# valeoai/PAFUSE

Measured on AMD Instinct MI355X. Metric: hypotheses/sec through DDIM loop (H3WB 133-kp, P=20, T=10), higher is better.
Workload: dtype bf16x3 (every fp32 GEMM operand as the exact sum of three bf16 slices, six bf16 MFMA products per fp32-equivalent product, fp32 accumulate; activations, LayerNorm, softmax, attention and everything in memory fp32; the residual stream stored centred on its row means)

## Files before the change

### pafuse_amd/csrc/kernels.hpp

```cpp
#pragma once
#include <hip/hip_runtime.h>
#include <stdint.h>

#include <utility>

namespace pafuse {

typedef float f32x16 __attribute__((ext_vector_type(16)));
typedef float f32x4 __attribute__((ext_vector_type(4)));

constexpr int BK = 32;
constexpr int LDK = 36;

typedef __bf16 bf16x8 __attribute__((ext_vector_type(8)));
__device__ __forceinline__ bf16x8 to_bf16x8(const f32x4 lo, const f32x4 hi) {
    bf16x8 v;
#pragma unroll
    for (int i = 0; i < 4; ++i) v[i] = (__bf16)lo[i], v[4 + i] = (__bf16)hi[i];
    return v;
}

#ifdef PAFUSE_MFMA_K8
typedef __bf16 bf16x4_t __attribute__((ext_vector_type(4)));
typedef short s16x4_t __attribute__((ext_vector_type(4)));
// ... 273 lines not shown
    float* out_head;
    float* ln_stats;
    const float* ln_in;
    const float* ln_s;
    const uint8_t* Ah;
    const uint8_t* Wh;
    uint8_t* out_h;
    uint8_t* out_xh;
    uint8_t* out_nh;
    const uint8_t* resid_h;
    const float* rowscale;
    int rs_temporal, rs_J, rs_FJ;
    float* out_pre;
    unsigned long long* stamps;
};

#ifdef PAFUSE_XQ_FENCE
struct XqFence {
    __device__ __forceinline__ XqFence() {
        if (PAFUSE_XQ_FENCE & 1) __builtin_amdgcn_fence(__ATOMIC_ACQUIRE, "agent");
        if (PAFUSE_XQ_FENCE & 4) {
            __builtin_amdgcn_fence(__ATOMIC_ACQUIRE, "agent");
            asm volatile("s_waitcnt vmcnt(0)" ::: "memory");
            __syncthreads();
        }
    }
    __device__ __forceinline__ ~XqFence() {
        if (PAFUSE_XQ_FENCE & 2) {
            asm volatile("s_waitcnt vmcnt(0)" ::: "memory");
            __builtin_amdgcn_fence(__ATOMIC_RELEASE, "agent");
            asm volatile("s_waitcnt vmcnt(0)" ::: "memory");
        }
    }
};
#define PAFUSE_XQ_GUARD() XqFence xq_fence_guard
#else
#define PAFUSE_XQ_GUARD()
#endif

#ifdef PAFUSE_STAMPS
__device__ __forceinline__ unsigned long long pafuse_stamp() {
    unsigned long long t;
    __builtin_amdgcn_sched_barrier(0);
    asm volatile("s_memtime %0\n\ts_waitcnt lgkmcnt(0)" : "=s"(t)::"memory");
    __builtin_amdgcn_sched_barrier(0);
    return t;
}
#ifndef PAFUSE_STAMP_SLOTS
#define PAFUSE_STAMP_SLOTS 4
#endif
#define PAFUSE_STAMP(i)                                                                         \
    if (p.stamps && (threadIdx.x & 63) == 0)                                                    \
    p.stamps[((size_t)blockIdx.x * (blockDim.x >> 6) + (threadIdx.x >> 6)) * PAFUSE_STAMP_SLOTS + (i)] = pafuse_stamp()
#else
#define PAFUSE_STAMP(i)
#endif

template <int WM, int WN, int NT>
struct GemmTile {
    static constexpr int NTHR = WM * WN * 64;
    static constexpr int BM = WM * 32;
    static constexpr int BN = WN * NT * 32;
    static constexpr int STAGE_FLOATS = (BM + BN) * LDK;
    static constexpr int W_ROW_SPLIT = WSPLIT_ROW_BYTES / 4;
    static constexpr int STAGE_FLOATS_SPLIT = BM * LDK + BN * W_ROW_SPLIT;
};

template <int WN, int NT, int BM, int EPI, int VEC = 0>
__device__ __forceinline__ void epilogue_row_per_lane(f32x16 (&acc)[NT], const GemmParams& p, const int64_t m0, const int n0,
                                                      const int wm, const int wn, const int r, const int h, float* smem,
                                                      const float ws = 1.0f) {
    constexpr int BNV = WN * NT * 32;
    auto vec4 = [&](const float* gptr, int slot, int n) -> f32x4 {
        if constexpr (VEC > 0) return *reinterpret_cast<const f32x4*>(smem + VEC + slot * BNV + (n - n0));
        else return *reinterpret_cast<const f32x4*>(gptr + n);
    };
    const int64_t m = m0 + wm * 32 + r;
    const bool live = m < p.M;
    const int64_t mo = (live ? m : p.M - 1) * p.N;
    const int nb = n0 + wn * NT * 32 + 4 * h;
    if constexpr (EPI == EPI_BIAS) {
        float rstd = 1.0f;
        if (p.ln_in) rstd = p.ln_in[2 * (live ? m : p.M - 1) + 1];
        rstd *= ws;
#pragma unroll
        for (int nt = 0; nt < NT; ++nt)
#pragma unroll
            for (int q = 0; q < 4; ++q) {
                const int n = nb + 32 * nt + 8 * q;
                const f32x4 b4 = *reinterpret_cast<const f32x4*>(p.bias + n);
                f32x4 v;
                if (p.ln_in) {
#pragma unroll
                    for (int e = 0; e < 4; ++e) v[e] = fmaf(rstd, acc[nt][4 * q + e], b4[e]);
                } else {
#pragma unroll
                    for (int e = 0; e < 4; ++e) v[e] = fmaf(acc[nt][4 * q + e], ws, b4[e]);
                }
#pragma unroll
                for (int e = 0; e < 4; ++e)
                    if (p.act) v[e] = gelu_erf(v[e]);
                if (live) *reinterpret_cast<f32x4*>(p.out + mo + n) = v;
            }
        PAFUSE_STAMP(2);
        return;
    } else {
        float* red = smem;
        const float invC = 1.0f / (float)p.N;
// ... 528 lines not shown
        if (m >= p.M) continue;
        float rstd = 1.0f;
        if (p.ln_in) rstd = p.ln_in[2 * m + 1];
        float* const orow = p.out + m * p.N + n0 + 4 * qd;
#pragma unroll
        for (int n = 0; n < NB; ++n) {
            const f32x4 b4 = *reinterpret_cast<const f32x4*>(p.bias + n0 + 16 * n + 4 * qd);
            f32x4 v;
            if (p.ln_in) {
#pragma unroll
                for (int e = 0; e < 4; ++e) v[e] = fmaf(rstd, acc[g][n][e], b4[e]);
            } else {
#pragma unroll
                for (int e = 0; e < 4; ++e) v[e] = acc[g][n][e] + b4[e];
            }
#pragma unroll
            for (int e = 0; e < 4; ++e)
                if (p.act) v[e] = gelu_erf(v[e]);
            if (p.dact_u) {
                const f32x4 u = *reinterpret_cast<const f32x4*>(p.dact_u + m * p.N + n0 + 4 * qd + 16 * n);
#pragma unroll
                for (int e = 0; e < 4; ++e) v[e] *= gelu_erf_grad(u[e]);
            }
            *reinterpret_cast<f32x4*>(orow + 16 * n) = v;
            if (p.out_act) {
#pragma unroll
                for (int e = 0; e < 4; ++e) v[e] = gelu_erf(v[e]);
                *reinterpret_cast<f32x4*>(p.out_act + m * p.N + n0 + 4 * qd + 16 * n) = v;
            }
        }
    }
}

template <int NB, int MINW>
__global__ void __launch_bounds__(256, MINW) gemm16_kernel(const GemmParams p) {
    PAFUSE_XQ_GUARD();
    extern __shared__ __attribute__((aligned(16))) float smem[];
    gemm16_tile<NB>(p, blockIdx.x, gridDim.x, smem);
}

template <int WM, int WN, int NT, int BKC = 32>
struct DmaTile {
    static_assert(BKC == 32 || BKC == 16, "chunk depth");
    static constexpr int NW = WM * WN, NTHR = NW * 64;
    static constexpr int BM = WM * 32, BN = WN * NT * 32;
    static constexpr int A_ROW = BKC * 4, W_ROW = BKC * 6;
    static constexpr int A_BYTES = BM * A_ROW, W_BYTES = BN * W_ROW, STAGE_BYTES = A_BYTES + W_BYTES;
    static constexpr int IA = A_BYTES / 1024, IW = W_BYTES / 1024;
    static constexpr int CNT = (IA + IW + NW - 1) / NW;
    static_assert(W_BYTES % 1024 == 0 && A_BYTES % 1024 == 0, "whole DMA pieces");
    static_assert(BKC == 16 || NW % 2 == 0, "the A swizzle of a wave's DMA lanes must not depend on the instruction index");
};

template <int... Is, class F>
__device__ __forceinline__ void static_for_impl(std::integer_sequence<int, Is...>, F&& f) {
    (f(std::integral_constant<int, Is>{}), ...);
}
template <int N, class F>
__device__ __forceinline__ void static_for(F&& f) {
    static_for_impl(std::make_integer_sequence<int, N>{}, f);
}

template <int OFF>
__device__ __forceinline__ u32x4 lds_read128(uint32_t addr) {
    u32x4 v;
    asm volatile("ds_read_b128 %0, %1 offset:%2" : "=v"(v) : "v"(addr), "i"(OFF));
    return v;
}

template <int N>
__device__ __forceinline__ void wait_vmcnt() {
    static_assert(N >= 0 && N < 64, "vmcnt immediate");
    asm volatile("s_waitcnt vmcnt(%0)" ::"n"(N) : "memory");
}

template <int WN, int NT, int BM, int NW, int NTH, bool HRES, int NSLICE = 2>
__device__ __forceinline__ void epilogue_rows_h(f32x16 (&acc)[NT], const GemmParams& p, const int64_t m0, const int n0, const int wm,
                                                const int wn, const int r, const int h, const int wave, const int lane, float* smem,
                                                const float ws);

template <int WM, int WN, int NT, int EPI, int NSTAGE, int ABL = 0, int BKC = 32, bool SLAB = true>
__device__ __forceinline__ void gemm_dma_tile(const GemmParams& p, const int b, const int nb, float* smem) {
    using T = DmaTile<WM, WN, NT, BKC>;
    constexpr int NW = T::NW, BM = T::BM, BN = T::BN, CNT = T::CNT, IA = T::IA, IW = T::IW;
    constexpr int NS2 = BKC / 16;
    constexpr int RPI = 1024 / T::A_ROW;
    constexpr int CPR = T::A_ROW / 16;
    static_assert(NSTAGE >= 2 && NSTAGE <= 4, "ring depth");
    static_assert(CNT * (NSTAGE - 1) < 64, "vmcnt range");
    uint8_t* const lds = reinterpret_cast<uint8_t*>(smem);
    const uint32_t lds0 = (uint32_t)(size_t)(__attribute__((address_space(3))) void*)smem;

    const int tid = threadIdx.x, lane = tid & 63;
    const int wave = __builtin_amdgcn_readfirstlane(tid >> 6);
    const int wm = wave / WN, wn = wave % WN;
    const int r = lane & 31, h = lane >> 5;
    const int tiles_n = p.N / BN;
    int tile;
    {
        const int xcd = b & 7, q = nb >> 3, rem = nb & 7;
        tile = (xcd < rem ? xcd * (q + 1) : rem * (q + 1) + (xcd - rem) * q) + (b >> 3);
    }
    const int tile_m = tile / tiles_n, tile_n = tile % tiles_n;
    const int64_t m0 = (int64_t)tile_m * BM;
    if (m0 >= p.M) return;
    PAFUSE_STAMP(0);
    const int n0 = tile_n * BN;
    const int K = p.K, nk = K / BKC;

    const float* Abase = p.A + m0 * K;
    const uint8_t* Wbase = p.Wsplit + (int64_t)n0 * T::W_ROW + lane * 16;
    const int64_t ws_chunk = (int64_t)p.N * T::W_ROW;
    const int sw_src = BKC == 32 ? (lane & 7) ^ ((4 * (wave & 1) + (lane >> 4)) & 7)
                                 : (lane & 3) ^ ((lane >> 4) & 3);
    int a_off[CNT];
#pragma unroll
    for (int j = 0; j < CNT; ++j) {
        int i = wave + j * NW;
        i = i < IA + IW ? i : IA + IW - 1;
        const int row = RPI * (i < IA ? i : 0) + lane / CPR;
        const int64_t lim = p.M - 1 - m0;
        const int grow = row < lim ? row : (int)lim;
        a_off[j] = grow * K + sw_src * 4;
    }
    auto issue_piece = [&](int kc, int st, int j) {
        if constexpr (ABL >= 2) return;
        uint8_t* const sa = lds + st * T::STAGE_BYTES;
        int i = wave + j * NW;
        i = i < IA + IW ? i : IA + IW - 1;
        if (i < IA)
            __builtin_amdgcn_global_load_lds((const __attribute__((address_space(1))) void*)(Abase + kc * BKC + a_off[j]),
                                             (__attribute__((address_space(3))) void*)(sa + i * 1024), 16, 0, 0);
        else
            __builtin_amdgcn_global_load_lds(
                (const __attribute__((address_space(1))) void*)(Wbase + kc * ws_chunk + (i - IA) * 1024),
                (__attribute__((address_space(3))) void*)(sa + T::A_BYTES + (i - IA) * 1024), 16, 0, 0);
    };
    auto issue = [&](int kc, int st) {
#pragma unroll
        for (int j = 0; j < CNT; ++j) issue_piece(kc, st, j);
    };

    f32x16 acc[NT];
#pragma unroll
    for (int nt = 0; nt < NT; ++nt)
#pragma unroll
        for (int i = 0; i < 16; ++i) acc[nt][i] = 0.f;

    const int sw = BKC == 32 ? (r >> 1) & 7 : (r >> 2) & 3;
    const int a_row = (wm * 32 + r) * T::A_ROW;
    int a_pos[4];
#pragma unroll
    for (int x = 0; x < 4; ++x) a_pos[x] = a_row + (((4 * (x >> 1) + 2 * h + (x & 1)) ^ sw) & (CPR - 1)) * 16;
    const int w_row = T::A_BYTES + (wn * NT * 32 + r) * T::W_ROW;
    const int w_sub[2] = {w_row + wsplit_sub_offset<BKC>(r, h), w_row + wsplit_sub_offset<BKC>(r, (2 + h) % (BKC / 8))};

    if constexpr (NS2 == 1 && NSTAGE == 3 && ABL != 1) {
        static_assert(NT >= 1, "groups");
#define PAFUSE_PIN_ACC(A) asm volatile("" : "+v"(A))
#define PAFUSE_PIN_PAIR(P) asm volatile("" : "+v"((P).x0), "+v"((P).x1), "+v"((P).s0), "+v"((P).s1), "+v"((P).s2))
        issue(0, 0);
        if (1 < nk) issue(1, 1);
        wait_vmcnt<0>();
        __builtin_amdgcn_s_barrier();
        u32x4 wf[2][3], cur[3], nxt[3];
        SplitPair sp[4];
        auto load_w = [&](auto SLOT, auto NTI, uint32_t stage_addr) {
            constexpr int slot = decltype(SLOT)::value, nti = decltype(NTI)::value;
            constexpr int full = nti * 32 * T::W_ROW;
            constexpr int off = full + 32 < 65536 ? full : 0;
            const uint32_t addr = stage_addr + (uint32_t)w_sub[0] + (uint32_t)(full - off);
            wf[slot][0] = lds_read128<off>(addr);
            wf[slot][1] = lds_read128<off + 16>(addr);
            wf[slot][2] = lds_read128<off + 32>(addr);
        };
        {
            u32x4 a_lo = lds_read128<0>(lds0 + (uint32_t)a_pos[0]);
            u32x4 a_hi = lds_read128<0>(lds0 + (uint32_t)a_pos[1]);
            load_w(std::integral_constant<int, 0>{}, std::integral_constant<int, 0>{}, lds0);
            asm volatile("s_waitcnt lgkmcnt(0)"
                         : "+v"(a_lo), "+v"(a_hi), "+v"(wf[0][0]), "+v"(wf[0][1]), "+v"(wf[0][2]));
#pragma unroll
            for (int q = 0; q < 4; ++q) {
                sp[q].x0 = __builtin_bit_cast(float, q < 2 ? a_lo[2 * q] : a_hi[2 * q - 4]);
                sp[q].x1 = __builtin_bit_cast(float, q < 2 ? a_lo[2 * q + 1] : a_hi[2 * q - 3]);
                sp[q].template stage<0>(), sp[q].template stage<1>(), sp[q].template stage<2>();
                sp[q].template stage<3>(), sp[q].template stage<4>();
                cur[0][q] = sp[q].s0, cur[1][q] = sp[q].s1, cur[2][q] = sp[q].s2;
            }
        }
        for (int kc = 0; kc < nk; ++kc) {
            if (kc > 0) {
                wait_vmcnt<0>();
                __builtin_amdgcn_s_barrier();
            }
            const bool refill = kc + 2 < nk;
            const int kn = kc + 2, stn = kn % 3;
            const uint32_t s_cur = lds0 + (uint32_t)((kc % 3) * T::STAGE_BYTES);
            const uint32_t s_nxt = lds0 + (uint32_t)(((kc + 1) % 3) * T::STAGE_BYTES);
            __builtin_amdgcn_s_setprio(1);
            u32x4 n_lo = lds_read128<0>(s_nxt + (uint32_t)a_pos[0]);
            u32x4 n_hi = lds_read128<0>(s_nxt + (uint32_t)a_pos[1]);
            static_for<NT>([&](auto G) {
                constexpr int g = decltype(G)::value;
                constexpr int q0 = ABL < 3 ? (4 * g) / NT : 0, q1 = ABL < 3 ? (4 * (g + 1)) / NT : 0;
                if constexpr (g + 1 < NT)
                    load_w(std::integral_constant<int, (g + 1) & 1>{}, std::integral_constant<int, g + 1>{}, s_cur);
                else
                    load_w(std::integral_constant<int, (g + 1) & 1>{}, std::integral_constant<int, 0>{}, s_nxt);
                if constexpr (g == 0) {
                    asm volatile("s_waitcnt lgkmcnt(3)" : "+v"(n_lo), "+v"(n_hi));
#pragma unroll
                    for (int q = 0; q < 4; ++q) {
                        sp[q].x0 = __builtin_bit_cast(float, q < 2 ? n_lo[2 * q] : n_hi[2 * q - 4]);
                        sp[q].x1 = __builtin_bit_cast(float, q < 2 ? n_lo[2 * q + 1] : n_hi[2 * q - 3]);
                    }
                } else {
                    asm volatile("s_waitcnt lgkmcnt(3)" : "+v"(wf[g & 1][0]), "+v"(wf[g & 1][1]), "+v"(wf[g & 1][2]));
                }
                const u32x4(&w)[3] = wf[g & 1];
                auto mm = [&](int wi, int ai) {
                    PAFUSE_PIN_ACC(acc[g]);
                    acc[g] = mfma_bf16_k16(__builtin_bit_cast(bf16x8, w[wi]), __builtin_bit_cast(bf16x8, cur[ai]), acc[g]);
                };
                auto pins = [&]() {
#pragma unroll
                    for (int q = q0; q < q1; ++q) PAFUSE_PIN_PAIR(sp[q]);
                };
                pins();
                mm(0, 2);
                {
                    constexpr int PER = (CNT + NT - 1) / NT, j0 = g * PER, j1 = (g + 1) * PER < CNT ? (g + 1) * PER : CNT;
                    if constexpr (j0 < j1 && ABL < 2) {
                        asm volatile("" ::: "memory");
                        if (refill) {
#pragma unroll
                            for (int j = j0; j < j1; ++j) issue_piece(kn, stn, j);
                        }
                        asm volatile("" ::: "memory");
                    }
                }
#pragma unroll
                for (int q = q0; q < q1; ++q) sp[q].template stage<0>();
                pins();
                mm(2, 0);
#pragma unroll
                for (int q = q0; q < q1; ++q) sp[q].template stage<1>();
                pins();
                mm(1, 1);
#pragma unroll
                for (int q = q0; q < q1; ++q) sp[q].template stage<2>();
                pins();
                mm(0, 1);
#pragma unroll
                for (int q = q0; q < q1; ++q) sp[q].template stage<3>();
                pins();
                mm(1, 0);
#pragma unroll
                for (int q = q0; q < q1; ++q) {
                    sp[q].template stage<4>();
                    nxt[0][q] = sp[q].s0, nxt[1][q] = sp[q].s1, nxt[2][q] = sp[q].s2;
                }
                pins();
                mm(0, 0);
            });
            asm volatile("s_waitcnt lgkmcnt(0)" : "+v"(wf[NT & 1][0]), "+v"(wf[NT & 1][1]), "+v"(wf[NT & 1][2]));
            if constexpr ((NT & 1) != 0) wf[0][0] = wf[1][0], wf[0][1] = wf[1][1], wf[0][2] = wf[1][2];
            if constexpr (ABL < 3) cur[0] = nxt[0], cur[1] = nxt[1], cur[2] = nxt[2];
            __builtin_amdgcn_s_setprio(0);
        }
#undef PAFUSE_PIN_ACC
#undef PAFUSE_PIN_PAIR
        wait_vmcnt<0>();
    } else {
    #pragma unroll
        for (int s = 0; s < NSTAGE - 1; ++s)
            if (s < nk) issue(s, s);

        for (int kc = 0; kc < nk; ++kc) {
            if (kc + NSTAGE - 2 < nk)
                wait_vmcnt<CNT*(NSTAGE - 2)>();
            else
                wait_vmcnt<0>();
            __builtin_amdgcn_s_barrier();
            if (kc == 0) { PAFUSE_STAMP(3); }
            const bool refill = kc + NSTAGE - 1 < nk;
            const int kn = kc + NSTAGE - 1, stn = kn % NSTAGE;
            const uint8_t* st = lds + (kc % NSTAGE) * T::STAGE_BYTES;
            if constexpr (ABL == 1) continue;
            constexpr int NG = NS2 * NT;
            __builtin_amdgcn_s_setprio(1);
    #define PAFUSE_PIN_ACC(A) asm volatile("" : "+v"(A))
    #define PAFUSE_PIN_PAIR(P) asm volatile("" : "+v"((P).x0), "+v"((P).x1), "+v"((P).s0), "+v"((P).s1), "+v"((P).s2))
            const uint32_t sbase = lds0 + (uint32_t)((kc % NSTAGE) * T::STAGE_BYTES);
            u32x4 wf[2][3];
            auto load_w = [&](auto G) {
                constexpr int g = decltype(G)::value;
                constexpr int full = (g % NT) * 32 * T::W_ROW;
                constexpr int off = full + 32 < 65536 ? full : 0;
                const uint32_t addr = sbase + (uint32_t)w_sub[g / NT] + (uint32_t)(full - off);
                wf[g & 1][0] = lds_read128<off>(addr);
                wf[g & 1][1] = lds_read128<off + 16>(addr);
                wf[g & 1][2] = lds_read128<off + 32>(addr);
            };
            u32x4 a_lo = lds_read128<0>(sbase + (uint32_t)a_pos[0]);
            u32x4 a_hi = lds_read128<0>(sbase + (uint32_t)a_pos[1]);
            load_w(std::integral_constant<int, 0>{});
            u32x4 b_lo, b_hi;
            if constexpr (NS2 == 2) {
                b_lo = lds_read128<0>(sbase + (uint32_t)a_pos[2]);
                b_hi = lds_read128<0>(sbase + (uint32_t)a_pos[3]);
                asm volatile("s_waitcnt lgkmcnt(5)" : "+v"(a_lo), "+v"(a_hi));
            } else {
                asm volatile("s_waitcnt lgkmcnt(3)" : "+v"(a_lo), "+v"(a_hi));
            }
            SplitPair sp[4];
            u32x4 cur[3], nxt[3];
    #pragma unroll
            for (int q = 0; q < 4; ++q) {
                sp[q].x0 = __builtin_bit_cast(float, q < 2 ? a_lo[2 * q] : a_hi[2 * q - 4]);
                sp[q].x1 = __builtin_bit_cast(float, q < 2 ? a_lo[2 * q + 1] : a_hi[2 * q - 3]);
                if constexpr (ABL >= 3) {
                    cur[0][q] = __builtin_bit_cast(uint32_t, sp[q].x0), cur[1][q] = __builtin_bit_cast(uint32_t, sp[q].x1);
                    cur[2][q] = cur[0][q];
                    continue;
                }
                sp[q].template stage<0>(), sp[q].template stage<1>(), sp[q].template stage<2>(), sp[q].template stage<3>();
                sp[q].template stage<4>();
                cur[0][q] = sp[q].s0, cur[1][q] = sp[q].s1, cur[2][q] = sp[q].s2;
            }
            static_for<NG>([&](auto G) {
                constexpr int g = decltype(G)::value;
                constexpr int nt = g % NT;
                constexpr bool SPL = g < NT && ABL < 3 && NS2 == 2;
                constexpr int q0 = SPL ? (4 * nt) / NT : 0, q1 = SPL ? (4 * (nt + 1)) / NT : 0;
                if constexpr (g + 1 < NG) {
                    load_w(std::integral_constant<int, g + 1>{});
                    if constexpr (g == 0 && NS2 == 2) {
                        asm volatile("s_waitcnt lgkmcnt(3)"
                                     : "+v"(wf[0][0]), "+v"(wf[0][1]), "+v"(wf[0][2]), "+v"(b_lo), "+v"(b_hi));
    #pragma unroll
                        for (int q = 0; q < 4; ++q) {
                            sp[q].x0 = __builtin_bit_cast(float, q < 2 ? b_lo[2 * q] : b_hi[2 * q - 4]);
                            sp[q].x1 = __builtin_bit_cast(float, q < 2 ? b_lo[2 * q + 1] : b_hi[2 * q - 3]);
                        }
                    } else {
                        asm volatile("s_waitcnt lgkmcnt(3)" : "+v"(wf[g & 1][0]), "+v"(wf[g & 1][1]), "+v"(wf[g & 1][2]));
                    }
                } else {
                    asm volatile("s_waitcnt lgkmcnt(0)" : "+v"(wf[g & 1][0]), "+v"(wf[g & 1][1]), "+v"(wf[g & 1][2]));
                }
                const u32x4(&w)[3] = wf[g & 1];
                auto mm = [&](int wi, int ai) {
                    PAFUSE_PIN_ACC(acc[nt]);
                    acc[nt] = mfma_bf16_k16(__builtin_bit_cast(bf16x8, w[wi]), __builtin_bit_cast(bf16x8, cur[ai]), acc[nt]);
                };
                auto pins = [&]() {
    #pragma unroll
                    for (int q = q0; q < q1; ++q) PAFUSE_PIN_PAIR(sp[q]);
                };
                pins();
                mm(0, 2);
                {
                    constexpr int PER = (CNT + NG - 1) / NG, j0 = g * PER, j1 = (g + 1) * PER < CNT ? (g + 1) * PER : CNT;
                    if constexpr (j0 < j1 && ABL < 2) {
                        asm volatile("" ::: "memory");
                        if (refill) {
    #pragma unroll
                            for (int j = j0; j < j1; ++j) issue_piece(kn, stn, j);
                        }
                        asm volatile("" ::: "memory");
                    }
                }
    #pragma unroll
                for (int q = q0; q < q1; ++q) sp[q].template stage<0>();
                pins();
                mm(2, 0);
    #pragma unroll
                for (int q = q0; q < q1; ++q) sp[q].template stage<1>();
                pins();
                mm(1, 1);
    #pragma unroll
                for (int q = q0; q < q1; ++q) sp[q].template stage<2>();
                pins();
                mm(0, 1);
    #pragma unroll
                for (int q = q0; q < q1; ++q) sp[q].template stage<3>();
                pins();
                mm(1, 0);
    #pragma unroll
                for (int q = q0; q < q1; ++q) {
                    sp[q].template stage<4>();
                    nxt[0][q] = sp[q].s0, nxt[1][q] = sp[q].s1, nxt[2][q] = sp[q].s2;
                }
                pins();
                mm(0, 0);
                if constexpr (g == NT - 1 && ABL < 3 && NS2 == 2) cur[0] = nxt[0], cur[1] = nxt[1], cur[2] = nxt[2];
                if constexpr (g == NT - 1 && ABL >= 3 && NS2 == 2) {
    #pragma unroll
                    for (int q = 0; q < 4; ++q)
                        cur[0][q] = cur[2][q] = __builtin_bit_cast(uint32_t, sp[q].x0), cur[1][q] = __builtin_bit_cast(uint32_t, sp[q].x1);
                }
            });
    #undef PAFUSE_PIN_ACC
    #undef PAFUSE_PIN_PAIR
            __builtin_amdgcn_s_setprio(0);
        }
    }
    PAFUSE_STAMP(1);
    __syncthreads();
    constexpr int VEC = EPI == EPI_BIAS ? 0 : (7 * BM * WN + 3) / 4 * 4;
    if constexpr (VEC > 0) {
        static_assert((size_t)(VEC + 5 * BN) * sizeof(float) <= (size_t)NSTAGE * T::STAGE_BYTES, "epilogue vectors must fit the ring");
        const float* const src[5] = {p.bias, p.post_w, p.post_b, p.next_w, p.next_b};
#pragma unroll
        for (int v = 0; v < 5; ++v)
            if (src[v])
                for (int i = tid; i < BN / 4; i += T::NTHR)
                    *reinterpret_cast<f32x4*>(smem + VEC + v * BN + 4 * i) = *reinterpret_cast<const f32x4*>(src[v] + n0 + 4 * i);
        __syncthreads();
    }
    if constexpr (ABL == 4) {
        float sacc = 0.f;
#pragma unroll
        for (int nt = 0; nt < NT; ++nt)
#pragma unroll
            for (int i = 0; i < 16; ++i) sacc += acc[nt][i];
        if (sacc == 123.456f) p.out[0] = sacc;
        return;
    }
    if constexpr (EPI == EPI_ROWLN && SLAB) {
        constexpr size_t RINGF = (size_t)NSTAGE * T::STAGE_BYTES / sizeof(float);
        constexpr auto need = [](int nth) { return (size_t)VEC + 5 * BN + (size_t)NW * 32 * (32 * nth + 4); };
        constexpr int NTH = (NT % 2 == 0 && need(2) <= RINGF) ? 2 : 1;
        static_assert(need(NTH) <= RINGF, "epilogue scratch must fit the ring");
        epilogue_rows_h<WN, NT, BM, NW, NTH, false, 2>(acc, p, m0, n0, wm, wn, r, h, wave, lane, smem, 1.0f);
    } else {
        epilogue_row_per_lane<WN, NT, BM, EPI, VEC>(acc, p, m0, n0, wm, wn, r, h, smem);
    }
}

template <int WM, int WN, int NT, int EPI, int NSTAGE, int MINW, int ABL = 0, int BKC = 32>
__global__ void __launch_bounds__(WM* WN * 64, MINW) gemm_dma_kernel(const GemmParams p) {
    PAFUSE_XQ_GUARD();
    extern __shared__ __attribute__((aligned(16))) float smem[];
    gemm_dma_tile<WM, WN, NT, EPI, NSTAGE, ABL, BKC>(p, blockIdx.x, gridDim.x, smem);
}

constexpr int GROUP_MAX = 4;
struct GroupedGemmParams {
    GemmParams p[GROUP_MAX];
    int first[GROUP_MAX + 1];
    int n;
};

template <int EPI>
__global__ void __launch_bounds__(256, 2) grouped_rowln_kernel(const GroupedGemmParams g) {
    PAFUSE_XQ_GUARD();
    extern __shared__ __attribute__((aligned(16))) float smem[];
    const int b = blockIdx.x;
    int s = 0;
#pragma unroll
    for (int i = 1; i < GROUP_MAX; ++i)
        if (i < g.n && b >= g.first[i]) s = i;
    const GemmParams& p = g.p[s];
    const int lb = b - g.first[s], nb = g.first[s + 1] - g.first[s];
    switch (p.N) {
        case 384: gemm_dma_tile<2, 2, 6, EPI, 2, 0, 16, false>(p, lb, nb, smem); break;
        case 256: gemm_dma_tile<2, 2, 4, EPI, 2, 0, 16, false>(p, lb, nb, smem); break;
        case 224: gemm_dma_tile<4, 1, 7, EPI, 2, 0, 16, false>(p, lb, nb, smem); break;
        default: break;
    }
}

struct AttnParams {
    const float* qkv;
    float* o;
    uint8_t* o_h;
    int64_t nseq;
    int L, C, heads, d;
    int64_t group, group_stride, seq_stride, tok_stride;
    float scale;
};

template <int ITEMS>
__device__ __forceinline__ void attn_item(int64_t i, int64_t nseq, int heads, int64_t& seq, int& head) {
    if (nseq % 8 == 0 && ((nseq / 8) * heads) % ITEMS == 0) {
        const int64_t blk = i / ITEMS;
        const int lo = (int)(blk % 8);
        const int64_t u = (blk / 8) * ITEMS + (i % ITEMS);
        head = (int)(u % heads);
        seq = (u / heads) * 8 + lo;
    } else {
        seq = i / heads;
        head = (int)(i % heads);
    }
}

template <int LP, int DP, int NW>
// ... 2494 lines not shown
```

### pafuse_amd/csrc/pafuse_hip.hip

```cpp
#include "../../include/pafuse_hip.h"

#include <hip/hip_runtime.h>

#include <algorithm>
#include <cmath>
#include <cstdarg>
#include <cstdio>
#include <cstdlib>
#include <cstring>

#include "kernels.hpp"
#include "hgemm.hpp"
#include "xgemm.hpp"
#include "sgemm.hpp"
#include "train_kernels.hpp"

using namespace pafuse;

namespace {

thread_local char g_err[512] = "";

int fail(int code, const char* fmt, ...) {
    va_list ap;
// ... 186 lines not shown
#define PAFUSE_STRIP_WGS_PER_CU 2
#endif
int device_cus() {
    static int cus[DeviceOnce::MAX_DEV] = {};
    int d = -1;
    if (hipGetDevice(&d) != hipSuccess || d < 0 || d >= DeviceOnce::MAX_DEV) return 256;
    if (!cus[d]) {
        int n = 0;
        if (hipDeviceGetAttribute(&n, hipDeviceAttributeMultiprocessorCount, d) != hipSuccess || n <= 0) n = 256;
        cus[d] = n;
    }
    return cus[d];
}

template <int NB, int FLAGS>
int launch_strip2(const GemmParams& p, hipStream_t s) {
    constexpr int RG = 2, NW = 4;
    using T = StripTile<NB, RG, NW, 2>;
    static_assert(T::LDS_BYTES <= 80 * 1024, "two workgroups per CU");
    if (!p.Wsplit) return fail(PAFUSE_E_ARG, "split-precision GEMM without a pre-split weight image");
    const int64_t tiles = ((p.M + T::BM - 1) / T::BM) * (p.N / T::BN);
    if (tiles <= 0 || tiles > 0x7fffffff) return fail(PAFUSE_E_ARG, "gemm grid out of range");
    int64_t grid = (int64_t)device_cus() * PAFUSE_STRIP_WGS_PER_CU / 8 * 8;
    if (grid >= tiles || grid <= 0) grid = tiles;
    return launch<sgemm2_kernel<NB, RG, NW, SEPI_BIAS, 2, FLAGS>>("sgemm2_kernel", (unsigned)grid, T::NTHR, T::LDS_BYTES, s, p);
}
bool strip2_ok(const GemmParams& p) {
    if ((p.out_act || p.dact_u) && (p.ln_in || p.act || (p.out_act && p.dact_u))) return false;
    return p.mode == MODE_BF16X3 && p.wlayout == WLAYOUT_M16 && p.K % 32 == 0 && p.K >= 128 && p.M > 0 &&
           p.M * (int64_t)p.N < (int64_t)1 << 31 && p.M * (int64_t)p.K < (int64_t)1 << 31 &&
           (p.N % 128 == 0 || p.N % 112 == 0 || p.N % 96 == 0);
}
template <int NB>
int launch_strip2_flags(const GemmParams& p, hipStream_t s) {
    const int flags = (p.ln_in ? 1 : 0) | (p.act ? 2 : 0) | (p.dact_u ? 4 : 0) | (p.out_act ? 8 : 0);
    switch (flags) {
        case 0: return launch_strip2<NB, 0>(p, s);
        case 1: return launch_strip2<NB, 1>(p, s);
        case 2: return launch_strip2<NB, 2>(p, s);
        case 3: return launch_strip2<NB, 3>(p, s);
        case 4: return launch_strip2<NB, 4>(p, s);
        case 8: return launch_strip2<NB, 8>(p, s);
        default: return fail(PAFUSE_E_ARG, "strip GEMM: epilogue options %d", flags);
    }
}
int strip2_bias(const GemmParams& p, hipStream_t s) {
    if (p.N % 128 == 0) return launch_strip2_flags<8>(p, s);
    if (p.N % 112 == 0) return launch_strip2_flags<7>(p, s);
    return launch_strip2_flags<6>(p, s);
}

int wsplit_chunk(int N, bool whole_row) { return (whole_row && (N == 384 || N == 288 || N == 256 || N == 224)) ? 16 : 32; }

template <int WM, int WN, int NT, int EPI, int NSTAGE, int MINW, int BKC = 32>
int launch_gemm_dma(const GemmParams& p, hipStream_t s) {
    using T = DmaTile<WM, WN, NT, BKC>;
    constexpr size_t lds = (size_t)NSTAGE * T::STAGE_BYTES;
    static_assert(lds <= 160 * 1024, "LDS budget");
    static_assert(EPI == EPI_BIAS || (size_t)7 * T::BM * WN * sizeof(float) <= lds, "cross-wave reduction scratch must fit");
    if (!p.Wsplit) return fail(PAFUSE_E_ARG, "split-precision GEMM without a pre-split weight image");
    if (p.K % BKC) return fail(PAFUSE_E_SHAPE, "split GEMM: K=%d is not a multiple of %d", p.K, BKC);
    const int64_t tiles = (p.M + T::BM - 1) / T::BM * (p.N / T::BN);
    if (tiles <= 0 || tiles > 0x7fffffff) return fail(PAFUSE_E_ARG, "gemm grid out of range");
    return launch<gemm_dma_kernel<WM, WN, NT, EPI, NSTAGE, MINW, 0, BKC>>("gemm_dma_kernel", (unsigned)tiles, T::NTHR, lds, s, p);
}

template <int WM, int WN, int NT, int EPI, int NSTAGE, int BKC, int MINW, bool HRES = false>
int launch_hgemm(const GemmParams& p, hipStream_t s) {
    using T = HTile<WM, WN, NT, BKC>;
    constexpr size_t lds = (size_t)NSTAGE * T::STAGE_BYTES;
    static_assert(lds <= 160 * 1024, "LDS budget");
    static_assert(EPI == EPI_BIAS || (size_t)7 * T::BM * WN * sizeof(float) <= lds, "cross-wave reduction scratch must fit");
    if (!p.Ah || !p.Wh) return fail(PAFUSE_E_ARG, "f16x2 GEMM without the H images of its operands");
    if (p.K % BKC || p.K <= 0 || p.N % T::BN) return fail(PAFUSE_E_SHAPE, "f16x2 GEMM: N=%d, K=%d do not fit the %d-column tile", p.N, p.K, T::BN);
    if (HRES && !p.resid_h) return fail(PAFUSE_E_ARG, "f16x2 whole-row GEMM: no H-image residual");
    const int64_t tiles = (p.M + T::BM - 1) / T::BM * (p.N / T::BN);
    if (tiles <= 0 || tiles > 0x7fffffff) return fail(PAFUSE_E_ARG, "gemm grid out of range");
    return launch<hgemm_kernel<WM, WN, NT, EPI, NSTAGE, BKC, MINW, HRES>>("hgemm_kernel", (unsigned)tiles, T::NTHR, lds, s, p);
}

bool hgemm_width(int C) { return C == 384 || C == 256 || C == 224; }
bool hgemm_plain_n(int N) { return N > 0 && (N % 128 == 0 || N % 224 == 0); }

int hgemm_bias(const GemmParams& p, hipStream_t s) {
    if (p.M <= 0) return PAFUSE_OK;
    if (p.N % 128 == 0) return launch_hgemm<4, 2, 2, EPI_BIAS, 3, 16, 2>(p, s);
    if (p.N % 224 == 0) return launch_hgemm<4, 1, 7, EPI_BIAS, 3, 16, 2>(p, s);
    return fail(PAFUSE_E_SHAPE, "f16x2 linear: N=%d must be a multiple of 128 or 224", p.N);
}

int hgemm_rowln(const GemmParams& p, hipStream_t s) {
    if (p.M <= 0) return PAFUSE_OK;
    if (p.resid_h)
        switch (p.N) {
            case 384: return launch_hgemm<4, 2, 6, EPI_ROWLN, 2, 32, 1, true>(p, s);
            case 256: return launch_hgemm<2, 2, 4, EPI_ROWLN, 2, 32, 2, true>(p, s);
            case 224: return launch_hgemm<4, 1, 7, EPI_ROWLN, 3, 16, 2, true>(p, s);
            default: break;
        }
    switch (p.N) {
        case 384: return launch_hgemm<4, 2, 6, EPI_ROWLN, 2, 32, 1>(p, s);
        case 256: return launch_hgemm<2, 2, 4, EPI_ROWLN, 2, 32, 2>(p, s);
        case 224: return launch_hgemm<4, 1, 7, EPI_ROWLN, 3, 16, 2>(p, s);
        default: return fail(PAFUSE_E_SHAPE, "no f16x2 whole-row kernel for channel width %d (have 224, 256, 384)", p.N);
    }
}

template <int WM, int WN, int NT, int EPI, int NSTAGE, int BKC, int MINW, bool HRES = false>
int launch_xgemm(const GemmParams& p, hipStream_t s) {
    using T = XTile<WM, WN, NT, BKC>;
    constexpr size_t lds = (size_t)NSTAGE * T::STAGE_BYTES;
    static_assert(lds <= 160 * 1024, "LDS budget");
    static_assert(EPI == EPI_BIAS || (size_t)7 * T::BM * WN * sizeof(float) <= lds, "cross-wave reduction scratch must fit");
    if (!p.Ah || !p.Wh) return fail(PAFUSE_E_ARG, "bf16x3 image GEMM without the X images of its operands");
    if (p.K % 32 || p.K <= 0 || p.N % T::BN) return fail(PAFUSE_E_SHAPE, "bf16x3 image GEMM: N=%d, K=%d do not fit the %d-column tile", p.N, p.K, T::BN);
    if (HRES && !p.resid_h) return fail(PAFUSE_E_ARG, "bf16x3 whole-row GEMM: no X-image residual");
    const int64_t tiles = (p.M + T::BM - 1) / T::BM * (p.N / T::BN);
// ... 61 lines not shown
    p.wlayout = WLAYOUT_PLAIN;
#endif
#ifndef PAFUSE_NO_STRIP
    if (strip2_ok(p)) return strip2_bias(p, s);
#endif
    if (p.mode == MODE_BF16X3 && p.wlayout == WLAYOUT_M16) {
        if (p.N % 128 == 0) return launch_gemm16<8, 3>(p, s);
        if (p.N % 96 == 0) return launch_gemm16<6, 3>(p, s);
        if (p.N % 112 == 0) return launch_gemm16<7, 3>(p, s);
        if (p.N % 64 == 0) return launch_gemm16<4, 4>(p, s);
        return launch_gemm16<2, 4>(p, s);
    }
    if (p.mode == MODE_BF16X3) {
        if (p.N % 128 == 0 && p.M >= 4096) return launch_gemm<4, 1, 4, EPI_BIAS, 1, PAFUSE_FC1_MINW, 0, 2>(p, s);
        if (p.N % 64 == 0) return launch_gemm<4, 1, 2, EPI_BIAS, 1, 4, 0, 2>(p, s);
        if (p.N % 96 == 0) return launch_gemm<4, 1, 3, EPI_BIAS, 1, 1, 1, 2>(p, s);
        return launch_gemm<4, 1, 1, EPI_BIAS, 1, 1, 0, 2>(p, s);
    }
    if (p.mode != MODE_F32) {
        if (p.N % 64 == 0) return launch_gemm<4, 1, 2, EPI_BIAS, 1, 5, 0, 1>(p, s);
        if (p.N % 96 == 0) return launch_gemm<4, 1, 3, EPI_BIAS, 1, 1, 1, 1>(p, s);
        return launch_gemm<4, 1, 1, EPI_BIAS, 1, 1, 0, 1>(p, s);
    }
    if (p.N % 64 == 0) return launch_gemm<4, 1, 2, EPI_BIAS, 1, 5>(p, s);
    if (p.N % 96 == 0) return launch_gemm<4, 1, 3, EPI_BIAS, 1, 1, 1>(p, s);
    return launch_gemm<4, 1, 1, EPI_BIAS, 1>(p, s);
}

template <int EPI>
int gemm_rowln_as(const GemmParams& p0, hipStream_t s) {
    GemmParams p = p0;
    if (p.mode == MODE_BF16X3 && (debug_f32_mask() & 2)) p.mode = MODE_F32;
    if (p.M <= 0) return PAFUSE_OK;
    if (p.K % BK || p.K <= 0) return fail(PAFUSE_E_SHAPE, "rowln: K=%d must be a positive multiple of 32", p.K);
    if (p.mode == MODE_F16X2 || p.mode == MODE_BF16X3_IMAGES) {
        if constexpr (EPI == EPI_ROWLN) return p.mode == MODE_F16X2 ? hgemm_rowln(p, s) : xgemm_rowln(p, s);
        else return fail(PAFUSE_E_ARG, "training has no image-pipeline kernels");
    }
    if constexpr (EPI == EPI_ROWLN_TRAIN) {
        if (p.mode == MODE_BF16X3) {
            switch (p.N) {
                case 384: return launch_gemm_dma<2, 2, 6, EPI, 2, 2, 16>(p, s);
                case 256: return launch_gemm_dma<2, 2, 4, EPI, 2, 2, 16>(p, s);
                case 224: if (p.M >= 4096) return launch_gemm_dma<4, 1, 7, EPI, 2, 2, 16>(p, s); break;
                default: break;
            }
            p.mode = MODE_F32;
        }
    }
    if constexpr (EPI == EPI_ROWLN) {
        if (p.mode == MODE_BF16X3) {
            switch (p.N) {
                case 384: return launch_gemm_dma<2, 2, 6, EPI, 2, 2, 16>(p, s);
                case 256: return launch_gemm_dma<2, 2, 4, EPI, 2, 2, 16>(p, s);
                case 288: return launch_gemm_dma<2, 3, 3, EPI, 2, 2, 16>(p, s);
                case 224:
                    return p.M >= 4096 ? launch_gemm_dma<4, 1, 7, EPI, 2, 2, 16>(p, s) : launch_gemm_dma<2, 1, 7, EPI, 2, 2, 16>(p, s);
                case 128: return launch_gemm<1, 4, 1, EPI, 1, 1, 1, 2>(p, s);
                case 64: return launch_gemm<1, 2, 1, EPI, 1, 1, 1, 2>(p, s);
                default: break;
            }
        } else if (p.mode != MODE_F32) {
            switch (p.N) {
                case 384: return launch_gemm<1, 4, 3, EPI, 1, 1, 1, 1>(p, s);
                case 288: return launch_gemm<1, 3, 3, EPI, 1, 1, 1, 1>(p, s);
                case 256: return launch_gemm<2, 2, 4, EPI, 1, 2, 1, 1>(p, s);
                case 224: return launch_gemm<1, 7, 1, EPI, 1, 1, 1, 1>(p, s);
                case 128: return launch_gemm<1, 4, 1, EPI, 1, 1, 1, 1>(p, s);
                case 64: return launch_gemm<1, 2, 1, EPI, 1, 1, 1, 1>(p, s);
                default: break;
            }
        }
    }
    switch (p.N) {
        case 384: return launch_gemm<1, 4, 3, EPI, 1, 1, 1>(p, s);
        case 288: return launch_gemm<1, 3, 3, EPI, 1, 1, 1>(p, s);
        case 256: return launch_gemm<2, 2, 4, EPI, 1, 2, 1>(p, s);
        case 224: return launch_gemm<1, 7, 1, EPI, 1, 1, 1>(p, s);
        case 128: return launch_gemm<1, 4, 1, EPI, 1, 1, 1>(p, s);
        case 64: return launch_gemm<1, 2, 1, EPI, 1, 1, 1>(p, s);
        default: return fail(PAFUSE_E_SHAPE, "no whole-row kernel for channel width %d (have 64,128,224,256,288,384)", p.N);
    }
}

int gemm_rowln(const GemmParams& p, hipStream_t s) { return gemm_rowln_as<EPI_ROWLN>(p, s); }
int gemm_rowln_train(const GemmParams& p, hipStream_t s) { return gemm_rowln_as<EPI_ROWLN_TRAIN>(p, s); }

bool group_ok_rowln(const GemmParams& p) {
    return p.mode == MODE_BF16X3 && p.Wsplit && (p.N == 384 || p.N == 256 || (p.N == 224 && p.M >= 4096)) && p.K % 16 == 0 && p.K > 0 &&
           !(debug_f32_mask() & 2);
}

template <bool ROWLN>
int gemm_group(const GemmParams* ps, int n, hipStream_t s, bool shared_grids) {
    bool ok = ROWLN && shared_grids && n >= 2 && n <= GROUP_MAX;
    for (int i = 0; i < n && ok; ++i) ok = ps[i].M > 0 && group_ok_rowln(ps[i]);
    if (!ok) {
        for (int i = 0; i < n; ++i) {
            const int rc = ROWLN ? gemm_rowln(ps[i], s) : gemm_bias(ps[i], s);
            if (rc) return rc;
        }
        return PAFUSE_OK;
    }
    int order[GROUP_MAX];
    double cost[GROUP_MAX];
    int64_t tiles[GROUP_MAX];
    for (int i = 0; i < n; ++i) {
// ... 2040 lines not shown
```

Before: 102.8.

## Use separate 3-deep weight and 2-deep activation LDS rings for N=256 row-LN GEMM

Adds an asymmetric DMA ring in which pre-split weight tiles get three LDS stages and activation tiles get two. The N=256 whole-row LayerNorm bf16x3 GEMM switches to this three-stage pipelined path. The aim is to hide weight-load latency with deeper prefetch while keeping the LDS footprint small enough for two workgroups per CU. The weight fragments for the first group are now loaded at the start of each iteration instead of prefetched from the next stage, and the vmcnt waits become partial. Optional timing-stamp macros are added as well, but they compile away by default.

```diff
diff --git a/pafuse_amd/csrc/kernels.hpp b/pafuse_amd/csrc/kernels.hpp
--- a/pafuse_amd/csrc/kernels.hpp
+++ b/pafuse_amd/csrc/kernels.hpp
@@ -349,8 +349,18 @@
 #define PAFUSE_STAMP(i)                                                                         \
     if (p.stamps && (threadIdx.x & 63) == 0)                                                    \
     p.stamps[((size_t)blockIdx.x * (blockDim.x >> 6) + (threadIdx.x >> 6)) * PAFUSE_STAMP_SLOTS + (i)] = pafuse_stamp()
+#define PAFUSE_TOP_DECL() unsigned long long top_t0 = 0, top_cyc = 0
+#define PAFUSE_TOP_BEGIN() top_t0 = pafuse_stamp()
+#define PAFUSE_TOP_END() top_cyc += pafuse_stamp() - top_t0
+#define PAFUSE_TOP_STORE()                                                                      \
+    if (PAFUSE_STAMP_SLOTS > 4 && p.stamps && (threadIdx.x & 63) == 0)                          \
+    p.stamps[((size_t)blockIdx.x * (blockDim.x >> 6) + (threadIdx.x >> 6)) * PAFUSE_STAMP_SLOTS + 4] = top_cyc
 #else
 #define PAFUSE_STAMP(i)
+#define PAFUSE_TOP_DECL()
+#define PAFUSE_TOP_BEGIN()
+#define PAFUSE_TOP_END()
+#define PAFUSE_TOP_STORE()
 #endif
 
 template <int WM, int WN, int NT>
@@ -985,6 +995,14 @@
     static_assert(BKC == 16 || NW % 2 == 0, "the A swizzle of a wave's DMA lanes must not depend on the instruction index");
 };
 
+template <class T, int NSW, int NSA>
+struct DmaRing {
+    static constexpr bool SPLIT = NSW != NSA;
+    static constexpr int BYTES = NSW * T::W_BYTES + NSA * T::A_BYTES;
+    static constexpr int a_off(int st) { return SPLIT ? NSW * T::W_BYTES + st * T::A_BYTES : st * T::STAGE_BYTES; }
+    static constexpr int w_off(int st) { return SPLIT ? st * T::W_BYTES : st * T::STAGE_BYTES + T::A_BYTES; }
+};
+
 template <int... Is, class F>
 __device__ __forceinline__ void static_for_impl(std::integer_sequence<int, Is...>, F&& f) {
     (f(std::integral_constant<int, Is>{}), ...);
@@ -1012,15 +1030,17 @@
                                                 const int wn, const int r, const int h, const int wave, const int lane, float* smem,
                                                 const float ws);
 
-template <int WM, int WN, int NT, int EPI, int NSTAGE, int ABL = 0, int BKC = 32, bool SLAB = true>
+template <int WM, int WN, int NT, int EPI, int NSTAGE, int ABL = 0, int BKC = 32, bool SLAB = true, int NSA = NSTAGE>
 __device__ __forceinline__ void gemm_dma_tile(const GemmParams& p, const int b, const int nb, float* smem) {
     using T = DmaTile<WM, WN, NT, BKC>;
+    using R = DmaRing<T, NSTAGE, NSA>;
     constexpr int NW = T::NW, BM = T::BM, BN = T::BN, CNT = T::CNT, IA = T::IA, IW = T::IW;
     constexpr int NS2 = BKC / 16;
     constexpr int RPI = 1024 / T::A_ROW;
     constexpr int CPR = T::A_ROW / 16;
     static_assert(NSTAGE >= 2 && NSTAGE <= 4, "ring depth");
     static_assert(CNT * (NSTAGE - 1) < 64, "vmcnt range");
+    static_assert(!R::SPLIT || (NS2 == 1 && NSTAGE == 3 && NSA == 2 && ABL != 1), "separate rings: the pipelined path only");
     uint8_t* const lds = reinterpret_cast<uint8_t*>(smem);
     const uint32_t lds0 = (uint32_t)(size_t)(__attribute__((address_space(3))) void*)smem;
 
@@ -1056,19 +1076,19 @@
         const int grow = row < lim ? row : (int)lim;
         a_off[j] = grow * K + sw_src * 4;
     }
-    auto issue_piece = [&](int kc, int st, int j) {
+    auto issue_piece2 = [&](int kc, int sta, int stw, int j) {
         if constexpr (ABL >= 2) return;
-        uint8_t* const sa = lds + st * T::STAGE_BYTES;
         int i = wave + j * NW;
         i = i < IA + IW ? i : IA + IW - 1;
         if (i < IA)
             __builtin_amdgcn_global_load_lds((const __attribute__((address_space(1))) void*)(Abase + kc * BKC + a_off[j]),
-                                             (__attribute__((address_space(3))) void*)(sa + i * 1024), 16, 0, 0);
+                                             (__attribute__((address_space(3))) void*)(lds + R::a_off(sta) + i * 1024), 16, 0, 0);
         else
             __builtin_amdgcn_global_load_lds(
                 (const __attribute__((address_space(1))) void*)(Wbase + kc * ws_chunk + (i - IA) * 1024),
-                (__attribute__((address_space(3))) void*)(sa + T::A_BYTES + (i - IA) * 1024), 16, 0, 0);
+                (__attribute__((address_space(3))) void*)(lds + R::w_off(stw) + (i - IA) * 1024), 16, 0, 0);
     };
+    auto issue_piece = [&](int kc, int st, int j) { issue_piece2(kc, st, st, j); };
     auto issue = [&](int kc, int st) {
 #pragma unroll
         for (int j = 0; j < CNT; ++j) issue_piece(kc, st, j);
@@ -1088,31 +1108,43 @@
     const int w_row = T::A_BYTES + (wn * NT * 32 + r) * T::W_ROW;
     const int w_sub[2] = {w_row + wsplit_sub_offset<BKC>(r, h), w_row + wsplit_sub_offset<BKC>(r, (2 + h) % (BKC / 8))};
 
+    PAFUSE_TOP_DECL();
     if constexpr (NS2 == 1 && NSTAGE == 3 && ABL != 1) {
+        constexpr bool ASYM = R::SPLIT;
+        constexpr int CA = IA / NW, CW = CNT - CA;
+        static_assert(!ASYM || (IA % NW == 0 && CW > 0 && CA + 2 * CW < 64), "every wave: CA A pieces, then CW W' pieces");
         static_assert(NT >= 1, "groups");
 #define PAFUSE_PIN_ACC(A) asm volatile("" : "+v"(A))
 #define PAFUSE_PIN_PAIR(P) asm volatile("" : "+v"((P).x0), "+v"((P).x1), "+v"((P).s0), "+v"((P).s1), "+v"((P).s2))
         issue(0, 0);
         if (1 < nk) issue(1, 1);
-        wait_vmcnt<0>();
+        if (ASYM && 1 < nk)
+            wait_vmcnt<ASYM ? CW : 0>();
+        else
+            wait_vmcnt<0>();
         __builtin_amdgcn_s_barrier();
         u32x4 wf[2][3], cur[3], nxt[3];
         SplitPair sp[4];
-        auto load_w = [&](auto SLOT, auto NTI, uint32_t stage_addr) {
+        const uint32_t w_frag = (uint32_t)(w_sub[0] - T::A_BYTES);
+        auto load_w = [&](auto SLOT, auto NTI, uint32_t slab_addr) {
             constexpr int slot = decltype(SLOT)::value, nti = decltype(NTI)::value;
             constexpr int full = nti * 32 * T::W_ROW;
             constexpr int off = full + 32 < 65536 ? full : 0;
-            const uint32_t addr = stage_addr + (uint32_t)w_sub[0] + (uint32_t)(full - off);
+            const uint32_t addr = slab_addr + w_frag + (uint32_t)(full - off);
             wf[slot][0] = lds_read128<off>(addr);
             wf[slot][1] = lds_read128<off + 16>(addr);
             wf[slot][2] = lds_read128<off + 32>(addr);
         };
         {
-            u32x4 a_lo = lds_read128<0>(lds0 + (uint32_t)a_pos[0]);
-            u32x4 a_hi = lds_read128<0>(lds0 + (uint32_t)a_pos[1]);
-            load_w(std::integral_constant<int, 0>{}, std::integral_constant<int, 0>{}, lds0);
-            asm volatile("s_waitcnt lgkmcnt(0)"
-                         : "+v"(a_lo), "+v"(a_hi), "+v"(wf[0][0]), "+v"(wf[0][1]), "+v"(wf[0][2]));
+            u32x4 a_lo = lds_read128<0>(lds0 + (uint32_t)R::a_off(0) + (uint32_t)a_pos[0]);
+            u32x4 a_hi = lds_read128<0>(lds0 + (uint32_t)R::a_off(0) + (uint32_t)a_pos[1]);
+            if constexpr (ASYM) {
+                asm volatile("s_waitcnt lgkmcnt(0)" : "+v"(a_lo), "+v"(a_hi));
+            } else {
+                load_w(std::integral_constant<int, 0>{}, std::integral_constant<int, 0>{}, lds0 + (uint32_t)R::w_off(0));
+                asm volatile("s_waitcnt lgkmcnt(0)"
+                             : "+v"(a_lo), "+v"(a_hi), "+v"(wf[0][0]), "+v"(wf[0][1]), "+v"(wf[0][2]));
+            }
 #pragma unroll
             for (int q = 0; q < 4; ++q) {
                 sp[q].x0 = __builtin_bit_cast(float, q < 2 ? a_lo[2 * q] : a_hi[2 * q - 4]);
@@ -1122,34 +1154,46 @@
                 cur[0][q] = sp[q].s0, cur[1][q] = sp[q].s1, cur[2][q] = sp[q].s2;
             }
         }
+        if constexpr (ASYM) __builtin_amdgcn_s_barrier();
         for (int kc = 0; kc < nk; ++kc) {
+            PAFUSE_TOP_BEGIN();
             if (kc > 0) {
-                wait_vmcnt<0>();
+                if (ASYM && kc + 1 < nk)
+                    wait_vmcnt<ASYM ? CW : 0>();
+                else
+                    wait_vmcnt<0>();
                 __builtin_amdgcn_s_barrier();
             }
+            if (kc == 0) { PAFUSE_STAMP(3); }
             const bool refill = kc + 2 < nk;
-            const int kn = kc + 2, stn = kn % 3;
-            const uint32_t s_cur = lds0 + (uint32_t)((kc % 3) * T::STAGE_BYTES);
-            const uint32_t s_nxt = lds0 + (uint32_t)(((kc + 1) % 3) * T::STAGE_BYTES);
+            const int kn = kc + 2;
+            const uint32_t s_cur = lds0 + (uint32_t)R::w_off(kc % 3);
+            const uint32_t s_nxt = lds0 + (uint32_t)R::w_off((kc + 1) % 3);
+            const uint32_t s_a = lds0 + (uint32_t)R::a_off((kc + 1) % NSA);
             __builtin_amdgcn_s_setprio(1);
-            u32x4 n_lo = lds_read128<0>(s_nxt + (uint32_t)a_pos[0]);
-            u32x4 n_hi = lds_read128<0>(s_nxt + (uint32_t)a_pos[1]);
+            u32x4 n_lo = lds_read128<0>(s_a + (uint32_t)a_pos[0]);
+            u32x4 n_hi = lds_read128<0>(s_a + (uint32_t)a_pos[1]);
+            if constexpr (ASYM) load_w(std::integral_constant<int, 0>{}, std::integral_constant<int, 0>{}, s_cur);
             static_for<NT>([&](auto G) {
                 constexpr int g = decltype(G)::value;
                 constexpr int q0 = ABL < 3 ? (4 * g) / NT : 0, q1 = ABL < 3 ? (4 * (g + 1)) / NT : 0;
+                constexpr int FLY = (g + 1 < NT || !ASYM) ? 3 : 0;
                 if constexpr (g + 1 < NT)
                     load_w(std::integral_constant<int, (g + 1) & 1>{}, std::integral_constant<int, g + 1>{}, s_cur);
-                else
+                else if constexpr (!ASYM)
                     load_w(std::integral_constant<int, (g + 1) & 1>{}, std::integral_constant<int, 0>{}, s_nxt);
                 if constexpr (g == 0) {
-                    asm volatile("s_waitcnt lgkmcnt(3)" : "+v"(n_lo), "+v"(n_hi));
+                    asm volatile("s_waitcnt lgkmcnt(%5)"
+                                 : "+v"(n_lo), "+v"(n_hi), "+v"(wf[0][0]), "+v"(wf[0][1]), "+v"(wf[0][2])
+                                 : "n"(FLY));
+                    PAFUSE_TOP_END();
 #pragma unroll
                     for (int q = 0; q < 4; ++q) {
                         sp[q].x0 = __builtin_bit_cast(float, q < 2 ? n_lo[2 * q] : n_hi[2 * q - 4]);
                         sp[q].x1 = __builtin_bit_cast(float, q < 2 ? n_lo[2 * q + 1] : n_hi[2 * q - 3]);
                     }
                 } else {
-                    asm volatile("s_waitcnt lgkmcnt(3)" : "+v"(wf[g & 1][0]), "+v"(wf[g & 1][1]), "+v"(wf[g & 1][2]));
+                    asm volatile("s_waitcnt lgkmcnt(%3)" : "+v"(wf[g & 1][0]), "+v"(wf[g & 1][1]), "+v"(wf[g & 1][2]) : "n"(FLY));
                 }
                 const u32x4(&w)[3] = wf[g & 1];
                 auto mm = [&](int wi, int ai) {
@@ -1168,7 +1212,7 @@
                         asm volatile("" ::: "memory");
                         if (refill) {
 #pragma unroll
-                            for (int j = j0; j < j1; ++j) issue_piece(kn, stn, j);
+                            for (int j = j0; j < j1; ++j) issue_piece2(kn, kn % NSA, kn % 3, j);
                         }
                         asm volatile("" ::: "memory");
                     }
@@ -1197,8 +1241,10 @@
                 pins();
                 mm(0, 0);
             });
-            asm volatile("s_waitcnt lgkmcnt(0)" : "+v"(wf[NT & 1][0]), "+v"(wf[NT & 1][1]), "+v"(wf[NT & 1][2]));
-            if constexpr ((NT & 1) != 0) wf[0][0] = wf[1][0], wf[0][1] = wf[1][1], wf[0][2] = wf[1][2];
+            if constexpr (!ASYM) {
+                asm volatile("s_waitcnt lgkmcnt(0)" : "+v"(wf[NT & 1][0]), "+v"(wf[NT & 1][1]), "+v"(wf[NT & 1][2]));
+                if constexpr ((NT & 1) != 0) wf[0][0] = wf[1][0], wf[0][1] = wf[1][1], wf[0][2] = wf[1][2];
+            }
             if constexpr (ABL < 3) cur[0] = nxt[0], cur[1] = nxt[1], cur[2] = nxt[2];
             __builtin_amdgcn_s_setprio(0);
         }
@@ -1211,6 +1257,7 @@
             if (s < nk) issue(s, s);
 
         for (int kc = 0; kc < nk; ++kc) {
+            PAFUSE_TOP_BEGIN();
             if (kc + NSTAGE - 2 < nk)
                 wait_vmcnt<CNT*(NSTAGE - 2)>();
             else
@@ -1283,6 +1330,7 @@
                 } else {
                     asm volatile("s_waitcnt lgkmcnt(0)" : "+v"(wf[g & 1][0]), "+v"(wf[g & 1][1]), "+v"(wf[g & 1][2]));
                 }
+                if constexpr (g == 0) { PAFUSE_TOP_END(); }
                 const u32x4(&w)[3] = wf[g & 1];
                 auto mm = [&](int wi, int ai) {
                     PAFUSE_PIN_ACC(acc[nt]);
@@ -1341,10 +1389,11 @@
         }
     }
     PAFUSE_STAMP(1);
+    PAFUSE_TOP_STORE();
     __syncthreads();
     constexpr int VEC = EPI == EPI_BIAS ? 0 : (7 * BM * WN + 3) / 4 * 4;
     if constexpr (VEC > 0) {
-        static_assert((size_t)(VEC + 5 * BN) * sizeof(float) <= (size_t)NSTAGE * T::STAGE_BYTES, "epilogue vectors must fit the ring");
+        static_assert((size_t)(VEC + 5 * BN) * sizeof(float) <= (size_t)R::BYTES, "epilogue vectors must fit the ring");
         const float* const src[5] = {p.bias, p.post_w, p.post_b, p.next_w, p.next_b};
 #pragma unroll
         for (int v = 0; v < 5; ++v)
@@ -1363,7 +1412,7 @@
         return;
     }
     if constexpr (EPI == EPI_ROWLN && SLAB) {
-        constexpr size_t RINGF = (size_t)NSTAGE * T::STAGE_BYTES / sizeof(float);
+        constexpr size_t RINGF = (size_t)R::BYTES / sizeof(float);
         constexpr auto need = [](int nth) { return (size_t)VEC + 5 * BN + (size_t)NW * 32 * (32 * nth + 4); };
         constexpr int NTH = (NT % 2 == 0 && need(2) <= RINGF) ? 2 : 1;
         static_assert(need(NTH) <= RINGF, "epilogue scratch must fit the ring");
@@ -1373,11 +1422,11 @@
     }
 }
 
-template <int WM, int WN, int NT, int EPI, int NSTAGE, int MINW, int ABL = 0, int BKC = 32>
+template <int WM, int WN, int NT, int EPI, int NSTAGE, int MINW, int ABL = 0, int BKC = 32, int NSA = NSTAGE>
 __global__ void __launch_bounds__(WM* WN * 64, MINW) gemm_dma_kernel(const GemmParams p) {
     PAFUSE_XQ_GUARD();
     extern __shared__ __attribute__((aligned(16))) float smem[];
-    gemm_dma_tile<WM, WN, NT, EPI, NSTAGE, ABL, BKC>(p, blockIdx.x, gridDim.x, smem);
+    gemm_dma_tile<WM, WN, NT, EPI, NSTAGE, ABL, BKC, true, NSA>(p, blockIdx.x, gridDim.x, smem);
 }
 
 constexpr int GROUP_MAX = 4;
diff --git a/pafuse_amd/csrc/pafuse_hip.hip b/pafuse_amd/csrc/pafuse_hip.hip
--- a/pafuse_amd/csrc/pafuse_hip.hip
+++ b/pafuse_amd/csrc/pafuse_hip.hip
@@ -262,17 +262,18 @@
 
 int wsplit_chunk(int N, bool whole_row) { return (whole_row && (N == 384 || N == 288 || N == 256 || N == 224)) ? 16 : 32; }
 
-template <int WM, int WN, int NT, int EPI, int NSTAGE, int MINW, int BKC = 32>
+template <int WM, int WN, int NT, int EPI, int NSTAGE, int MINW, int BKC = 32, int NSA = NSTAGE>
 int launch_gemm_dma(const GemmParams& p, hipStream_t s) {
     using T = DmaTile<WM, WN, NT, BKC>;
-    constexpr size_t lds = (size_t)NSTAGE * T::STAGE_BYTES;
+    constexpr size_t lds = DmaRing<T, NSTAGE, NSA>::BYTES;
     static_assert(lds <= 160 * 1024, "LDS budget");
+    static_assert(NSA == NSTAGE || MINW * lds <= 160 * 1024, "the asymmetric ring exists to keep MINW workgroups on a CU");
     static_assert(EPI == EPI_BIAS || (size_t)7 * T::BM * WN * sizeof(float) <= lds, "cross-wave reduction scratch must fit");
     if (!p.Wsplit) return fail(PAFUSE_E_ARG, "split-precision GEMM without a pre-split weight image");
     if (p.K % BKC) return fail(PAFUSE_E_SHAPE, "split GEMM: K=%d is not a multiple of %d", p.K, BKC);
     const int64_t tiles = (p.M + T::BM - 1) / T::BM * (p.N / T::BN);
     if (tiles <= 0 || tiles > 0x7fffffff) return fail(PAFUSE_E_ARG, "gemm grid out of range");
-    return launch<gemm_dma_kernel<WM, WN, NT, EPI, NSTAGE, MINW, 0, BKC>>("gemm_dma_kernel", (unsigned)tiles, T::NTHR, lds, s, p);
+    return launch<gemm_dma_kernel<WM, WN, NT, EPI, NSTAGE, MINW, 0, BKC, NSA>>("gemm_dma_kernel", (unsigned)tiles, T::NTHR, lds, s, p);
 }
 
 template <int WM, int WN, int NT, int EPI, int NSTAGE, int BKC, int MINW, bool HRES = false>
@@ -440,7 +441,7 @@
         if (p.mode == MODE_BF16X3) {
             switch (p.N) {
                 case 384: return launch_gemm_dma<2, 2, 6, EPI, 2, 2, 16>(p, s);
-                case 256: return launch_gemm_dma<2, 2, 4, EPI, 2, 2, 16>(p, s);
+                case 256: return launch_gemm_dma<2, 2, 4, EPI, 3, 2, 16, 2>(p, s);
                 case 288: return launch_gemm_dma<2, 3, 3, EPI, 2, 2, 16>(p, s);
                 case 224:
                     return p.M >= 4096 ? launch_gemm_dma<4, 1, 7, EPI, 2, 2, 16>(p, s) : launch_gemm_dma<2, 1, 7, EPI, 2, 2, 16>(p, s);
```

Result: no change. 102.8 (-0.0%).
